# avaneev/r8brain-free-src

Measured on NVIDIA H100. Metric: input Msamples/s (Mrops), fp64 44100->96000, higher is better.
Workload: dtype f64

## Files before the change

### r8brain-free-src_b200/csrc/r8b_capi.cu

```cuda
#include "../../include/r8bgpu.h"

#include <algorithm>
#include <climits>
#include <cmath>
#include <cstddef>
#include <cstdio>
#include <cstdlib>
#include <cstring>
#include <functional>
#include <map>
#include <memory>
#include <optional>
#include <string>
#include <utility>
#include <vector>

#include "r8b_codec.cuh"
#include "r8b_dither.cuh"
#include "r8b_dsd.cuh"
#include "r8b_dsdmod.cuh"
#include "r8b_fft.cuh"
#include "r8b_hosttab.h"
#include "r8b_kernels.h"
#include "r8b_multi.h"
// ... 117 lines not shown
        return &h_;
    }

  private:
    H h_ = nullptr;
};
using Event = Handle<cudaEvent_t, cudaEventDestroy>;
using Stream = Handle<cudaStream_t, cudaStreamDestroy>;

template <class T>
struct RecRing {
    DevBuf<T> d;
    PinBuf<T> h[2];
    Event ev[2];
    int cur = 0;

    bool create(unsigned long long& charge, size_t n, const char* dev_what, const char* host_what, const char* ev_what)
    {
        if (!d.alloc(charge, n, dev_what)) return false;
        for (int k = 0; k < 2; k++)
            if (!h[k].alloc(n, host_what) || !cuda_ok(cudaEventCreateWithFlags(ev[k].put(), cudaEventDisableTiming), ev_what))
                return false;
        return true;
    }
    T* next(const char* what)
    {
        cur ^= 1;
        return cuda_ok(cudaEventSynchronize(ev[cur]), what) ? (T*) h[cur] : nullptr;
    }
    T* host() const { return h[cur]; }
    bool upload(size_t first, size_t n, cudaStream_t st, const char* what)
    {
        return cuda_ok(cudaMemcpyAsync(d + first, h[cur] + first, n * sizeof(T), cudaMemcpyHostToDevice, st), what) &&
               cuda_ok(cudaEventRecord(ev[cur], st), what);
    }
};

struct StageDev {
    int fft_log2 = 0, lg = 0, virt_up = 1;
    double nyq_gain = 0.0;
    DevBuf<double2> spec;
    DevBuf<double2> tw;
    bool large = false;
    DevBuf<double2> tw_m;
    DevBuf<double2> scratch;
    long long scratch_pairs = 0;
    DevBuf<double> bank;
    int frac_tile_fixed = 0;
    int frac_tile_ragged = 0;
    std::string unfused_variant;
    DevBuf<double> ring;
    long long ring_cap = 0;
    bool fused_with_next = false;
    bool fused_into_prev = false;
    DevBuf<int> phase_off;
    DevBuf<int> phase_row;
    DevBuf<double> gbank;
    DevBuf<int> goff;
    int gbank_len = 0, gbank_smem_len = 0, smaxp = 0, ir = 8;
    int yl = 0, yr = 0, ysh = 31, span_max = 0, bank_in_smem = 0;
    RecRing<int> ft_dp;
    RecRing<double> ft_fpos;
    int casc_len = 0;
    HbCascadeParams up_casc;
    int up_casc_smem = 0;
    int down_casc_len = 0;
    HbDownCascParams down_casc;
    int down_casc_smem = 0;
    int casc_variant = 0;
    DevBuf<double2> tw_tab;
    DevBuf<double2> c_tab;
    DevBuf<double2> cd_tab;
    DevBuf<double2> cs_tab;
    DevBuf<double2> c_tab_v1;
    bool bank_frag_order = false;
    bool f2_ok = false;
    bool f2_poly = false;
    bool f2_copy = false;
    FusedGeom fgeom;
    FusedVariant last_variant;
};

struct FusedKnobs {
    int f2_flags = 6;
    bool f2_flags_env = false;
    bool v1 = false;
    bool no_fusion = false;
    bool poly_v2 = false;
};

FusedKnobs fused_knobs_env()
{
    FusedKnobs k;
    if (const char* e = getenv("R8BGPU_F2_FLAGS")) {
        k.f2_flags = atoi(e);
        k.f2_flags_env = true;
    }
    k.v1 = getenv("R8BGPU_FUSED_V1") != nullptr;
    k.no_fusion = getenv("R8BGPU_NO_FUSION") != nullptr;
    k.poly_v2 = getenv("R8BGPU_POLY_V2") != nullptr;
    return k;
}

struct FusedPlan {
    FusedGeom geom;
    bool copy = false;
    bool poly_v2 = false;
    bool cs = false;
    bool whole = false;
    GroupBank tc, fma;
    bool tc_fits = false, fma_fits = false;
    bool tc_bank = false;
    bool bank_in_smem = false;
    int kernel = R8BGPU_FUSED_NONE;
};

FusedPlan plan_fused_stage(const std::vector<StageDesc>& st, size_t i, const FusedKnobs& k)
{
    FusedPlan fp;
    const StageDesc& s = st[i];
    if (s.kind != ST_BLOCKCONV) return fp;
    fp.whole = i + 1 < st.size() && st[i + 1].kind == ST_FRAC_WHOLE;
    if (fp.whole) {
        const StageDesc& f = st[i + 1];
        auto f2_fits = [](const GroupBank& gb) {
            return fused2_smem_bytes(gb.n_groups * gb.smaxp * gb.ir, false, false) <= kFused2SmemMax && gb.n_groups <= 192;
        };
        fp.tc = build_group_bank(f, 8, true);
        fp.fma = build_group_bank(f, choose_group_ir(f), false);
        fp.tc_fits = f2_fits(fp.tc);
        fp.fma_fits = f2_fits(fp.fma);
    }
    if (i + 1 < st.size() && !k.no_fusion) {
        fp.geom = fused_geometry(s, st[i + 1]);
        if (fp.geom.ok && fp.geom.up == 1 && (k.v1 || !(k.f2_flags & 4) || !fp.tc_fits)) fp.geom = FusedGeom();
    }
    const bool fused = fp.geom.ok;
    if (fused && st[i + 1].kind == ST_FRAC_POLY && fp.geom.up == 2 && (k.f2_flags & 4) && !k.v1 && k.poly_v2 &&
        (st[i + 1].bank.filter_len & 1) == 0 && st[i + 1].bank.filter_len <= 32)
        fp.poly_v2 = true;
    if (!fused && s.up == 2 && s.down == 1 && !s.block_exact && !k.no_fusion && !k.v1) {
        const BcTile bt = blockconv_tile(s);
        if (!bt.large && 2 * (4096 - 2 * bt.lg) >= 2048) fp.copy = true;
    }
    if ((fused && fp.geom.up == 2) || fp.copy) fp.cs = fused2_cs_fits(fused ? fused2_bank_doubles_max(st[i + 1]) : 0);
    if (fused && fp.whole) {
        const bool want_f2 = !k.v1;
        fp.tc_bank = want_f2 && (k.f2_flags & 4) && fp.tc_fits;
        const GroupBank& B = fp.tc_bank ? fp.tc : fp.fma;
        fp.bank_in_smem = fused_smem_bytes(B.n_groups * B.smaxp * B.ir) <= 220 * 1024;
        if (want_f2 && (fp.tc_bank || fp.fma_fits)) fp.kernel = fp.tc_bank ? R8BGPU_FUSED_F2_TC : R8BGPU_FUSED_F2_FMA;
        else fp.kernel = fp.bank_in_smem ? R8BGPU_FUSED_V1_SMEM : R8BGPU_FUSED_V1_GLOBAL;
    } else if (fused) {
        fp.kernel = R8BGPU_FUSED_ORDER2;
    } else if (fp.copy) {
        fp.kernel = R8BGPU_FUSED_F2_COPY;
    }
    return fp;
}

struct HbKnobs {
    bool no_cascade = false;
    bool no_last2 = false;
    int up_budget = 7000;
    int down_budget = 6400;
};

// ... 154 lines not shown
    std::vector<int> part_of, row_of;
    std::vector<std::vector<int>> chans;
    int max_out = 0, flush_max_out = 0;
    std::vector<Stream> streams;
    std::vector<Event> done;
    Event fork;
    RecRing<MapRec> map;
    DevBuf<unsigned char> raw_in;
    DevBuf<unsigned char> raw_out;
};

static_assert(sizeof(DitherCfg) == sizeof(r8bgpu_dither) && offsetof(DitherCfg, taps) == offsetof(r8bgpu_dither, taps),
              "DitherCfg mirrors r8bgpu_dither");
struct DitherState {
    std::vector<DitherCfg> cfg;
    bool any = false;
    DevBuf<DitherCfg> d_cfg;
    DevBuf<double> d_err;
    RecRing<DitherRec> rec;
    std::vector<long long> m;
    DevBuf<DitherCall> d_call;
    DevBuf<double> d_zero;
};

struct StateStaging {
    DevBuf<unsigned char> d_blob;
    PinBuf<unsigned char> h_blob;
    DevBuf<unsigned char> d_aux;
};

struct DsdOutState {
    DevBuf<DsdModState> d_state;
    std::vector<int> pend;
    RecRing<DsdModRec> rec;
    DevBuf<double> d_y;
    size_t y_cap = 0;
    DevBuf<unsigned char> d_in;
    DevBuf<unsigned char> d_bytes;
};

struct r8bgpu_batch {
    std::optional<DeviceGuard> releasing;
    unsigned long long dev_bytes = 0;
    std::unique_ptr<DsdOutState> dsd;
    std::unique_ptr<StateStaging> stx;
    std::unique_ptr<DitherState> dith;
    std::unique_ptr<ShardFront> front;
    std::unique_ptr<MixedFront> mixed;
    const Plan* plan = nullptr;
    Plan plan_copy;
    int n_ch = 0;
    int device = 0;
    cudaStream_t stream = nullptr;
    Schedule sched;
    bool diverged = false;
    RaggedSchedule rag;
    RecRing<RaggedRec> rec;
    bool links_fresh = false;
    std::vector<StageDev> dev;
    std::vector<StageCall> calls;
    unsigned long long launches = 0;
    bool timing = false;
    struct EvPair {
        int stage;
        Event a, b;
    };
    std::vector<EvPair> events;
    std::vector<double> stage_ms;
    std::vector<unsigned long long> stage_launches;
    DevBuf<double> st_in;
    DevBuf<double> st_out;
    DevBuf<unsigned char> raw_in;
    DevBuf<unsigned char> raw_out;
    DevBuf<double> fl_out;
    DevBuf<unsigned char> fl_raw;
    size_t fl_cap = 0;
    std::vector<long long> pass_n;
    std::vector<double> trim;
    Stream s_h2d, s_d2h, s_comp;
    int host_groups = 1;
    std::vector<Event> ev_h2d, ev_k;
    DevBuf<unsigned long long> prof;
    int n_sm = 0;
    int f2_flags = 6;
    bool f2_flags_env = false;
    unsigned long long prof_ctas = 0;
    bool prof_v2 = false;

    ~r8bgpu_batch()
    {
        if (front) {
            front->pool.reset();
            return;
        }
        releasing.emplace(device);
        if (mixed) {
            cudaStreamSynchronize(stream);
            mixed->parts.clear();
        }
        unsigned long long h[10] = {};
        if (prof != nullptr && cudaDeviceSynchronize() == cudaSuccess &&
            cudaMemcpy(h, prof, sizeof h, cudaMemcpyDeviceToHost) == cudaSuccess) {
            if (prof_v2) {
                const double n = prof_ctas ? (double) prof_ctas : 1.0;
                const unsigned long long tot = h[0] + h[1] + h[2] + h[3] + h[4] + h[7] + h[8];
                auto line = [&](const char* nm, double v) {
                    fprintf(stderr, "  %-26s %9.0f  (%4.1f %%)\n", nm, v / n, tot ? 100.0 * v / tot : 0.0);
                };
                fprintf(stderr, "[r8bgpu profile] k_up2_frac2 phases, mean clk per tile (one half-CTA) over %llu tiles:\n", prof_ctas);
                line("A_wait landed tile", (double) h[0]);
                line("A_work gather+fwd1", (double) h[1]);
                line("A_bar", (double) h[2]);
                line("B fwd2+fwd3", (double) h[3]);
                line("C+D split*G, inverse", (double) h[4]);
                line("E interp", (double) (h[7] + h[8]));
                line("  E_work mean over warps", h[5] / 8.0);
                line("  E_work max over warps", (double) h[6]);
                line("  E_bar (thread 0)", (double) h[7]);
                fprintf(stderr, "  %-26s %9.0f\n", "total", tot / n);
            } else {
                static const char* nm[8] = {"gather+fwd1", "fwd2", "fwd3", "C(split*G)", "inv1", "inv2", "inv3+ystore", "interp"};
                unsigned long long tot = 0;
                for (int i = 0; i < 8; i++) tot += h[i];
                fprintf(stderr, "[r8bgpu profile] k_up2_frac phases, mean clk per CTA over %llu CTAs:\n", prof_ctas);
                for (int i = 0; i < 8; i++)
                    fprintf(stderr, "  %-12s %9.0f  (%4.1f %%)\n", nm[i], prof_ctas ? (double) h[i] / prof_ctas : 0.0,
                            tot ? 100.0 * h[i] / tot : 0.0);
                if (h[8] + h[9] > 0)
                    fprintf(stderr, "  order-2 bank, clk per CTA: 4-output groups %.0f, queued single outputs %.0f\n",
                            (double) h[8] / prof_ctas, (double) h[9] / prof_ctas);
            }
        }
    }
};


static const std::vector<std::unique_ptr<r8bgpu_batch>>* sub_batches(const r8bgpu_batch* b)
{
    return b->front ? &b->front->shards : b->mixed ? &b->mixed->parts : nullptr;
}

static std::vector<const r8bgpu_batch*> plan_batches(const r8bgpu_batch* b)
{
    const auto* subs = sub_batches(b);
    if (subs == nullptr) return {b};
    std::vector<const r8bgpu_batch*> v;
    for (const auto& sb : *subs) v.push_back(sb.get());
    return v;
}

struct Slot {
    r8bgpu_batch* b;
    int row, sub;
};

static Slot slot_of(const r8bgpu_batch* b, int c)
{
    if (b->front) {
        const std::vector<int>& ch0 = b->front->ch0;
        const int s = (int) (std::upper_bound(ch0.begin(), ch0.end(), c) - ch0.begin()) - 1;
        return Slot{b->front->shards[(size_t) s].get(), c - ch0[(size_t) s], s};
    }
    if (b->mixed) {
        const int p = b->mixed->part_of[(size_t) c];
        return Slot{b->mixed->parts[(size_t) p].get(), b->mixed->row_of[(size_t) c], p};
    }
    return Slot{const_cast<r8bgpu_batch*>(b), c, 0};
}

struct ChannelGroup {
    r8bgpu_batch* b;
    std::vector<int> rows, idx;
};

static std::vector<ChannelGroup> group_channels(const r8bgpu_batch* b, const int* channels, int n)
{
    const auto* subs = sub_batches(b);
    std::vector<ChannelGroup> g(subs ? subs->size() : 1);
    for (size_t k = 0; k < g.size(); k++) g[k].b = subs ? (*subs)[k].get() : const_cast<r8bgpu_batch*>(b);
    for (int i = 0; i < n; i++) {
        const Slot s = slot_of(b, channels[i]);
        g[(size_t) s.sub].rows.push_back(s.row);
        g[(size_t) s.sub].idx.push_back(i);
    }
    return g;
}

template <class T>
static std::vector<T> gather(const T* v, const std::vector<int>& idx)
{
    std::vector<T> out;
    out.reserve(idx.size());
    for (int i : idx) out.push_back(v[i]);
    return out;
// ... 1314 lines not shown
                const double outs = 2.0 * p.span / ratio + 4.0;
                const int row_words = 6 * p.flen;
                p.poly_row_stride = 3 * p.flen + ((row_words % 8) == 4 ? 0 : 2);
                const int cap = (224 * 1024 - fused_smem_bytes(0) - fused_poly_queue_bytes()) /
                                (p.poly_row_stride * (int) sizeof(double));
                const double up = fr * p.fracs * outs + 4.0, dn = (1.0 - fr) * p.fracs * outs + 4.0;
                const double need = up < dn ? up : dn;
                const int chunks = (int) ceil(need / cap);
                if (cap >= 8 && chunks <= 4) {
                    p.poly_dir = up < dn ? 1 : -1;
                    p.poly_rows_cap = cap;
                    p.poly_chunks = chunks < 1 ? 1 : chunks;
                    const long long nn = llround(ratio);
                    if (nn >= 1 && nn <= 3 && !getenv("R8BGPU_POLY_SINGLE")) {
                        p.poly_n = (int) nn;
                        p.ysh = 4;
                    }
                }
            }
            if (p.poly_chunks < 1) p.poly_chunks = 1;
            if (b->prof == nullptr && getenv("R8BGPU_PROFILE") && b->prof.alloc(b->dev_bytes, 10, "profile: cudaMalloc"))
                cudaMemset(b->prof, 0, 10 * sizeof(unsigned long long));
            p.prof = b->prof;
#ifdef R8BGPU_EXPERIMENTS
            if (const char* e = getenv("R8BGPU_DEBUG")) p.debug = atoi(e);
#endif
            if (b->prof) {
                b->prof_ctas += (unsigned long long) (v2 ? p.n_tiles : (p.n_tiles + 1) / 2) * nch;
                b->prof_v2 = v2;
            }
            if (v2) {
                p.n_ch = nch;
                p.flags = b->f2_flags;
                p.tw_tab = d.tw_tab;
                p.c_tab = d.c_tab;
                p.cd_tab = d.cd_tab;
                p.cs_tab = d.cs_tab;
                p.up = d.fgeom.up;
                p.ylen = d.fgeom.up * 4096;
                if (!fd.bank_frag_order) p.flags &= ~4;
                if (!b->f2_flags_env && !v2_poly && p.up != 1 && p.cs_tab != nullptr && (p.flags & 4)) p.flags |= 1;
                const bool cs = p.cs_tab != nullptr;
                p.stage_off = (p.ir == 8 && !(p.flags & 4) && fused2_smem_bytes(p.gbank_smem_len, cs, true) <= kFused2SmemMax &&
                               !getenv("R8BGPU_NO_STAGE")) ? fused2_stage_off(p.gbank_smem_len, cs) : 0;
                if (v2_poly) {
                    p.ysh = 31;
                    p.gbank_smem_len = 0;
                    p.stage_off = 0;
                }
                p.glog = v2_poly ? 0 : fused2_choose_glog(p.span, f.in_step, f.out_step, p.ir);
                p.mbu = v2_poly ? 0 : fused2_choose_mbu(p.span, f.in_step, f.out_step);
                launch_up2_frac2(p, src, dst, b->n_sm, st, &b->dev[i].last_variant);
            } else {
                p.c_tab = d.c_tab_v1;
                launch_up2_frac(p, src, dst, nch, st, &b->dev[i].last_variant);
            }
            b->launches++;
        } else
        switch (s.kind) {
        case ST_BLOCKCONV: {
            if (d.f2_copy) {
                FusedParams fp;
                memset(&fp, 0, sizeof fp);
                fp.mode = 2;
                fp.e0 = c.e0;
                fp.e1 = c.e1;
                fp.p_lo = c.e0 & ~1LL;
                fp.p_hi = c.e1;
                fused2_tiles(fp, d.fgeom, i == 0 ? (int) (c.n0 & 1) : -1);
                fp.lg = d.lg;
                fp.ysh = 31;
                fp.spec = d.spec;
                fp.tw = d.tw;
                fp.tw_tab = d.tw_tab;
                fp.c_tab = d.c_tab;
                fp.cd_tab = d.cd_tab;
                fp.cs_tab = d.cs_tab;
                fp.up = 2;
                fp.ylen = 8192;
                fp.ir = 8;
                fp.out_step = 8;
                fp.smaxp = 4;
                fp.n_ch = nch;
                fp.flags = b->f2_flags & 2;
                launch_up2_frac2(fp, src, dst, b->n_sm, st, &b->dev[i].last_variant);
                b->launches++;
                break;
            }
            BlockConvParams p;
            blockconv_call_fields(p, s, d.virt_up, d.lg, d.fft_log2, c.e0, c.e1);
            p.nyq_gain = d.nyq_gain;
            p.spec = d.spec;
            p.tw = d.tw;
            if (d.large) {
                BcLargeParams lp;
                lp.bc = p;
                lp.tw_m = d.tw_m;
                lp.scratch = d.scratch;
                const long long pairs = (p.n_tiles + 1) / 2;
                lp.group_ch = (int) std::max(1LL, std::min((long long) nch, d.scratch_pairs / std::max(1LL, pairs)));
                b->launches += (unsigned long long) launch_blockconv_large(lp, src, dst, nch, st);
                if (p.n_tiles > 0 && nch > 0)
                    b->dev[i].unfused_variant = bcl_variant(p, lp.group_ch, nch);
                break;
            }
            launch_blockconv(p, src, dst, nch, st);
            if (p.n_tiles > 0 && nch > 0) b->dev[i].unfused_variant = blockconv_variant(p);
            b->launches++;
            break;
        }
        case ST_FRAC_WHOLE:
        case ST_FRAC_POLY: {
            FracParams p;
            memset(&p, 0, sizeof p);
            p.flen = s.bank.filter_len;
            p.fll = s.bank.filter_len / 2 - 1;
            p.e0 = c.e0;
            p.e1 = c.e1;
            p.bank = d.bank;
            p.in_step = s.in_step;
            p.out_step = s.out_step;
            p.fracs = s.bank.fracs;
            p.ssr = s.kind == ST_FRAC_POLY ? c.ssr : s.src_rate;
            p.dsr = s.kind == ST_FRAC_POLY ? c.dsr : s.dst_rate;
            p.in_counter0 = c.in_counter0;
            p.in_pos_int0 = c.in_pos_int0;
            p.in_pos_shift = c.in_pos_shift;
            p.fpos0 = c.fpos0;
            p.p0 = c.p0;
            p.pos_dp = d.ft_dp.d;
            p.pos_fpos = d.ft_fpos.d;
            const int tile = d.frac_tile_fixed > 0 ? d.frac_tile_fixed : frac_tile(p.ssr / p.dsr, p.flen);
            if (s.kind == ST_FRAC_WHOLE) launch_frac_whole(p, tile, src, dst, nch, st);
            else launch_frac_poly(p, tile, src, dst, nch, st);
            if (p.e1 > p.e0 && nch > 0) b->dev[i].unfused_variant = frac_variant(s, tile);
            b->launches++;
            break;
        }
        case ST_HBUP:
        case ST_HBDOWN: {
            HbParams p;
            memset(&p, 0, sizeof p);
            p.ntaps = s.hb_taps;
            p.e0 = c.e0;
            p.e1 = c.e1;
            for (int k = 0; k < s.hb_taps; k++) p.taps[k] = s.hb[(size_t) k];
            if (s.kind == ST_HBUP) launch_hbup(p, src, dst, nch, st);
            else launch_hbdown(p, src, dst, nch, st);
            b->launches++;
            break;
        }
        }
        time_end(b, ev, st);
    }
    if (l > 0) {
        const StageCall& c0 = calls[0];
        const StageDev& d0 = b->dev[0];
        long long from = c0.n1 - d0.ring_cap;
        if (from < c0.n0) from = c0.n0;
        launch_save_tail(d_in, (long long) in_stride, c0.n0, from, c0.n1, d0.ring + (long long) ch0 * d0.ring_cap, d0.ring_cap,
                         d0.ring_cap - 1, nch, st, tio.in_fmt, tio.in_scale);
        b->launches++;
    }
}


static bool has_fasttiming(const Plan& P)
// ... 2983 lines not shown
```

### r8brain-free-src_b200/csrc/r8b_fused2.cu

```cuda
#include "r8b_kernels.h"

#include <algorithm>
#include <cstdint>
#include <type_traits>

#include "r8b_fused2_core.cuh"
#include "r8b_poly.cuh"

namespace r8bgpu {

namespace {

using namespace f2;

constexpr int NT2 = 2 * HT;
constexpr int STAGE_UP = fft_pad(FN);

__device__ __forceinline__ void bar_half(int h) { asm volatile("bar.sync %0, 256;" ::"r"(h + 1) : "memory"); }
__device__ __forceinline__ uint32_t smem_u32(const void* p) { return (uint32_t) __cvta_generic_to_shared(p); }
__device__ __forceinline__ void mbar_init(unsigned long long* b, int count)
{
    asm volatile("mbarrier.init.shared::cta.b64 [%0], %1;" ::"r"(smem_u32(b)), "r"(count) : "memory");
}
__device__ __forceinline__ void fence_mbar_init() { asm volatile("fence.mbarrier_init.release.cluster;" ::: "memory"); }
// ... 39 lines not shown
    const int n_j = s_i[0], c_cnt = s_i[1], jshift = s_i[2];
    const int n_groups = (p.out_step + 7) / 8;
    const int n_gt = (n_groups + G::GL - 1) / G::GL;
    const int gt = task % n_gt, chunk = task / n_gt;
    const int wrow = (lane ^ ((lane >> 2) & 1)) * 8, wsw = (lane >> 1) & 3;
#pragma unroll
    for (int q = 0; q < IQ2; q++) {
        const int cq = chunk * G::CYC + q * G::CL;
        if (cq > c_cnt) break;
#pragma unroll
        for (int i = 0; i < 4; i++)
            *reinterpret_cast<double2*>(stg + wrow + 2 * (i ^ wsw)) = make_double2(acc[2 * i][q], acc[2 * i + 1][q]);
        __syncwarp();
        const int ci = lane & 3;
#pragma unroll
        for (int t = 0; t < 4; t++) {
            const int R = (lane & ~3) + t;
            const double2 v = *reinterpret_cast<const double2*>(stg + (R ^ ((R >> 2) & 1)) * 8 + 2 * (ci ^ ((R >> 1) & 3)));
            const int c = cq + (R & (G::CL - 1));
            const int grp = gt * G::GL + (R >> (5 - GLOG));
            if (c > c_cnt || grp >= n_groups) continue;
            const int r0 = p.delta + grp * 8;
            const int j = c * p.out_step + r0 + jshift + 2 * ci;
            double* o = s_o + j;
            const bool in0 = (p.wrap || r0 + 2 * ci < p.out_step) && j >= 0 && j < n_j;
            const bool in1 = (p.wrap || r0 + 2 * ci + 1 < p.out_step) && j + 1 >= 0 && j + 1 < n_j;
            if (in0 && in1 && ((reinterpret_cast<unsigned long long>(o) & 15) == 0)) {
                *reinterpret_cast<double2*>(o) = v;
            } else {
                if (in0) o[0] = v.x;
                if (in1) o[1] = v.y;
            }
        }
        __syncwarp();
    }
}

}

__device__ __forceinline__ void dmma884(double& c0, double& c1, double a, double b)
{
    asm volatile("mma.sync.aligned.m8n8k4.row.col.f64.f64.f64.f64 {%0,%1}, {%2}, {%3}, {%0,%1};" : "+d"(c0), "+d"(c1) : "d"(a), "d"(b));
}

template <int KW>
__device__ __forceinline__ void dmma16(double (&c)[4], const double (&a)[KW / 2], const double (&b)[KW / 4])
{
    if constexpr (KW == 16)
        asm volatile("mma.sync.aligned.m16n8k16.row.col.f64.f64.f64.f64 {%0,%1,%2,%3}, {%4,%5,%6,%7,%8,%9,%10,%11}, "
                     "{%12,%13,%14,%15}, {%0,%1,%2,%3};"
                     : "+d"(c[0]), "+d"(c[1]), "+d"(c[2]), "+d"(c[3])
                     : "d"(a[0]), "d"(a[1]), "d"(a[2]), "d"(a[3]), "d"(a[4]), "d"(a[5]), "d"(a[6]), "d"(a[7]), "d"(b[0]), "d"(b[1]),
                       "d"(b[2]), "d"(b[3]));
    else if constexpr (KW == 8)
        asm volatile("mma.sync.aligned.m16n8k8.row.col.f64.f64.f64.f64 {%0,%1,%2,%3}, {%4,%5,%6,%7}, {%8,%9}, {%0,%1,%2,%3};"
                     : "+d"(c[0]), "+d"(c[1]), "+d"(c[2]), "+d"(c[3])
                     : "d"(a[0]), "d"(a[1]), "d"(a[2]), "d"(a[3]), "d"(b[0]), "d"(b[1]));
    else
        asm volatile("mma.sync.aligned.m16n8k4.row.col.f64.f64.f64.f64 {%0,%1,%2,%3}, {%4,%5}, {%6}, {%0,%1,%2,%3};"
                     : "+d"(c[0]), "+d"(c[1]), "+d"(c[2]), "+d"(c[3])
                     : "d"(a[0]), "d"(a[1]), "d"(b[0]));
}

template <int IRV, bool PADV, int GLOG, bool TC, int UP = 2, bool COPY = false, bool POLY = false, bool CS = false, bool LIN = false>
__global__ void __launch_bounds__(NT2, 1) k_up2_frac2(const __grid_constant__ FusedParams p, const __grid_constant__ SrcView src,
                                                      const __grid_constant__ DstView dst)
{
    extern __shared__ __align__(128) double2 smem[];
    double2* const tw2 = smem + 2 * FPL2;
    double2* const twf = tw2 + 256;
    double* const sbank = reinterpret_cast<double*>(twf + 256);
    const int n_groups = (p.out_step + IRV - 1) / IRV, esz = p.smaxp * IRV;
    const int n_bank = (COPY || POLY) ? 0 : n_groups;
    static_assert(!CS || UP == 2, "the symmetric spectrum table is the 2x pair's");
    double2* const scs = reinterpret_cast<double2*>(sbank + ((n_bank * esz + 1) & ~1));
    TileEntry* const tab = reinterpret_cast<TileEntry*>(reinterpret_cast<char*>(smem) + p.tab_off);
    __shared__ __align__(8) unsigned long long mb[5];
    __shared__ TileEntry s_te[2];
    __shared__ int s_goff[192];

    const int tid = threadIdx.x, h = tid >> 8, ht = tid & (HT - 1), lane = tid & 31, wh = ht >> 5;
    double2* const buf = smem + h * FPL2;
    const int n_units = p.n_tiles * p.n_ch;
    const bool pingpong = (p.flags & 1) != 0, tma_in = (p.flags & 2) != 0;

    if (tid == 0) {
#pragma unroll
        for (int i = 0; i < 5; i++) mbar_init(&mb[i], 1);
        fence_mbar_init();
    }
    if (!COPY && !POLY && tid < n_groups) s_goff[tid] = __ldg(&p.goff[p.delta + tid * IRV]);
    if (!COPY)
        for (int i = tid; i < p.n_tab; i += NT2) tab[i] = tile_entry(p, dst.base, i);
    __syncthreads();
    if (tid == 0) {
        mbar_expect_tx(&mb[0], (uint32_t) (512 * sizeof(double2) + (size_t) n_bank * esz * sizeof(double) +
                                           (CS ? CS_PAIRS * sizeof(double2) : 0)));
        bulk_g2s(tw2, p.tw_tab, 512 * sizeof(double2), &mb[0]);
        if (CS) bulk_g2s(scs, p.cs_tab, CS_PAIRS * sizeof(double2), &mb[0]);
        for (int g = 0; g < n_bank; g++)
            bulk_g2s(sbank + g * esz, p.gbank + (long long) (p.delta + g * IRV) * esz, (uint32_t) (esz * sizeof(double)), &mb[0]);
        mbar_arrive(&mb[3]);
    }

    const int stride = 2 * (int) gridDim.x;
    int u = 2 * (int) blockIdx.x + h;
    uint32_t par_in = 0, par_turn = 0;
    Tile t;
    int path = -1;
    auto tile_src = [&](const Tile& tt) { return tile_run(src, tt); };
    if (u < n_units) {
        t = tile_of(p, u);
        path = tile_input_path(src, t);
        if (path == 2 && !tma_in) path = 1;
        if (path == 2 && ht == 0) {
            mbar_expect_tx(&mb[1 + h], FM * sizeof(double));
            bulk_g2s(buf + STAGE_UP, tile_src(t), FM * sizeof(double), &mb[1 + h]);
        }
    }
    mbar_wait(&mb[0], 0);

#ifdef R8BGPU_PHASE_TIMERS
    __shared__ unsigned long long s_emax[2];
    if (ht == 0) s_emax[h] = 0;
    long long t_prev = clock64();
#define R8B_TICK(i)                                                                  \
    if (p.prof != nullptr && ht == 0) {                                              \
        const long long t_now = clock64();                                           \
        atomicAdd(&p.prof[i], (unsigned long long) (t_now - t_prev));                \
        t_prev = t_now;                                                              \
    }
#else
#define R8B_TICK(i)
#endif
    for (; u < n_units; u += stride) {
        Tile tn = t;
        int pathn = -1;
        if (u + stride < n_units) {
            tn = tile_of(p, u + stride);
            pathn = tile_input_path(src, tn);
            if (pathn == 2 && !tma_in) pathn = 1;
            if ((pathn == 1 || pathn == 2) && ht == 0) bulk_prefetch_l2(reinterpret_cast<const void*>(reinterpret_cast<unsigned long long>(tile_src(tn)) & ~15ull),
                                                        FM * sizeof(double));
        }
        {
            double2 v[8];
            if (path == 2) {
                R8B_TICK(1)
                mbar_wait(&mb[1 + h], par_in);
                R8B_TICK(0)
                par_in ^= 1;
                const double2* st = buf + STAGE_UP;
#pragma unroll
                for (int j = 0; j < 8; j++) v[j] = st[ht + 256 * j];
            } else {
                gather_tile(v, src, t, path, ht);
            }
            fwd_pass1_r8(v, buf, tw2, twf, ht);
        }
        if (!COPY && u - t.ch * p.n_tiles >= p.n_tab && ht == HT - 1) s_te[h] = tile_entry(p, dst.base, u - t.ch * p.n_tiles);
        R8B_TICK(1)
        bar_half(h);
        R8B_TICK(2)
        constexpr bool fuse_c = (UP == 2);
        if (ht < FN / 16) {
            fwd_pass<256>(buf, tw2, ht);
            __syncwarp();
            if constexpr (fuse_c) fwd_pass16_skew(buf, ht);
            else fwd_pass<16>(buf, tw2, ht);
        }
        bar_half(h);
        R8B_TICK(3)
        if constexpr (fuse_c) {
            double2 z1[8], z2[8];
            cd1_load(buf, ht, z1, z2);
            bar_half(h);
            if constexpr (CS) cd1s_compute(scs, __ldg(&p.cs_tab[CS_PAIRS + ht]), __ldg(&p.cs_tab[CS_PAIRS + HT + ht]), buf, ht, z1, z2);
            else cd1_compute(p, buf, ht, z1, z2);
        } else {
            double2 z1[4], z2[4], ze = make_double2(0.0, 0.0);
            c_load(buf, ht, z1, z2);
            if (ht == 0) ze = buf[fft_pad(slot_of<FN>(FN / 2))];
            bar_half(h);
#pragma unroll
            for (int i = 0; i < 4; i++) c1_pair_tab(p, buf, ht, i, z1[i], z2[i]);
            if (ht == 0) c1_pair_mid(p, buf, ze);
            bar_half(h);
        }
        if constexpr (UP == 2) {
            __syncwarp();
            inv_pass<256>(buf, tw2, ht);
            bar_half(h);
            {
                double2 v[16];
                inv3_load(buf, tw2, twf, ht, v);
                bar_half(h);
                y_store<PADV>(buf, v, ht, t.w, p.ysh);
            }
        } else {
            if (ht < FN / 16) {
                inv_pass<16>(buf, tw2, ht);
                __syncwarp();
                inv_pass<256>(buf, tw2, ht);
            }
            bar_half(h);
            {
                double2 v[8];
                inv1_last_load(buf, tw2, twf, ht, v);
                bar_half(h);
                y_store1<PADV>(buf, v, ht, t.w, p.ysh);
            }
        }
        bar_half(h);
        R8B_TICK(4)
        if (pingpong) {
            mbar_wait(&mb[3 + h], par_turn);
            par_turn ^= 1;
        }
#ifdef R8BGPU_PHASE_TIMERS
        const long long t_e0 = clock64();
#endif
        {
            const double* yb = reinterpret_cast<const double*>(buf);
            const int ti = u - t.ch * p.n_tiles;
            const TileEntry& te = ti < p.n_tab ? tab[ti] : s_te[h];
            const int* si = te.s;
            const long long drow = (long long) t.ch * dst.stride;
            if constexpr (POLY) {
                const int ka = si[0], kb = si[1], N = p.poly_n, flen = p.flen, ksteps = (flen + 3) >> 2;
                const int row = lane >> 2, kq = lane & 3;
                const unsigned full = 0xffffffffu;
                const int n_rounds = (kb - ka + 31) >> 5;
                int cached_row = -2;
                double bq[8];
                auto load_b = [&](int fmin) {
                    cached_row = fmin;
                    int brow = fmin + (row & 1);
                    if (brow > p.fracs) brow = p.fracs;
                    const double* __restrict__ br = p.bank + (long long) brow * 3 * flen + (row >> 1);
#pragma unroll
                    for (int ks = 0; ks < 8; ks++) {
// ... 98 lines not shown
                    for (int i = ht; i < cnt; i += HT) orow[(d0 + i) & dst.mask] = yb[off + i];
                }
            } else if constexpr (TC) {
                MmaTile mt;
                mt.load(te, drow);
                const int n_mu = mt.n_j > 0 ? mma_units(p, mt.c_cnt) : 0, smaxp = p.smaxp;
                double* const so = dst.ptr + drow + (te.off & dst.mask);
                constexpr int WS = HT / 32;
                auto run_units = [&](auto mb_tag) {
                    constexpr int MB = decltype(mb_tag)::value;
                    MmaUnit mu;
                    mu.set(wh, n_groups);
                    for (int unit = wh; unit < n_mu; unit += WS) {
                        int yo[2 * MB];
                        const int goff = s_goff[mu.g];
#pragma unroll
                        for (int i = 0; i < 2 * MB; i++) yo[i] = mma_a_index(p, mt, mu, goff, i, lane);
                        const double* const gb = sbank + mma_b_index(p, mu, lane);
                        double acc[MB][4];
#pragma unroll
                        for (int m = 0; m < MB; m++) acc[m][0] = acc[m][1] = acc[m][2] = acc[m][3] = 0.0;
                        auto kchunk = [&](auto kw_tag, int k0) {
                            constexpr int KW = decltype(kw_tag)::value;
                            double b[KW / 4];
#pragma unroll
                            for (int i = 0; i < KW / 4; i++) b[i] = gb[8 * k0 + 32 * i];
#pragma unroll
                            for (int m = 0; m < MB; m++) {
                                double a[KW / 2];
#pragma unroll
                                for (int i = 0; i < KW / 2; i++) {
                                    const int yi = yo[2 * m + (i & 1)] + k0 + 4 * (i >> 1);
                                    a[i] = PADV ? yb[ylay(yi, p.ysh)] : yb[yi];
                                }
                                dmma16<KW>(acc[m], a, b);
                            }
                        };
                        using K16 = std::integral_constant<int, 16>;
                        const int k16 = smaxp & ~15;
#pragma unroll 1
                        for (int k0 = 0; k0 < k16; k0 += 16) kchunk(K16(), k0);
                        if (smaxp & 8) kchunk(std::integral_constant<int, 8>(), k16);
                        if (smaxp & 4) kchunk(std::integral_constant<int, 4>(), k16 + (smaxp & 8));
#pragma unroll
                        for (int m = 0; m < MB; m++) {
                            mma_store<LIN>(p, dst, t.ch, mt, so, mu, 2 * m, lane, acc[m][0], acc[m][1]);
                            mma_store<LIN>(p, dst, t.ch, mt, so, mu, 2 * m + 1, lane, acc[m][2], acc[m][3]);
                        }
                        mu.advance(WS, n_groups);
                    }
                };
                switch (mma_mbu(p)) {
                case 2: run_units(std::integral_constant<int, 1>()); break;
                case 4: run_units(std::integral_constant<int, 2>()); break;
                default: run_units(std::integral_constant<int, 3>()); break;
                }
            } else if (si[0] > 0) {
                const int n_tasks = TaskGeom<IRV, GLOG>::n_tasks(p, si[1]);
                double* const stg = p.stage_off > 0 ? reinterpret_cast<double*>(smem) + p.stage_off + (tid >> 5) * 256 : nullptr;
                double* const so = dst.ptr + drow + (te.off & dst.mask);
                for (int task = wh; task < n_tasks; task += HT / 32) {
                    TaskGeom<IRV, GLOG> g;
                    g.set(p, s_goff, task, lane);
                    int yo[IQ2];
                    interp_windows<IRV, GLOG>(p, g, si, yo);
                    double acc[IRV][IQ2];
                    interp_acc<IRV, PADV>(yb, sbank + g.grp * esz, yo, p.smaxp, p.ysh, acc);
                    if (IRV == 8 && dst.mask == -1 && stg != nullptr) {
                        if constexpr (IRV == 8) interp_store_staged<GLOG>(p, si, so, stg, task, lane, acc);
                    } else {
                        interp_store_direct<IRV, GLOG>(p, dst, t.ch, g, si, so, acc);
                    }
                }
            }
        }
#ifdef R8BGPU_PHASE_TIMERS
        if (p.prof != nullptr && lane == 0) {
            const unsigned long long dt = (unsigned long long) (clock64() - t_e0);
            atomicAdd(&p.prof[5], dt);
            atomicMax(&s_emax[h], dt);
        }
#endif
        R8B_TICK(8)
        bar_half(h);
        R8B_TICK(7)
#ifdef R8BGPU_PHASE_TIMERS
        if (p.prof != nullptr && ht == 0) {
            atomicAdd(&p.prof[6], s_emax[h]);
            s_emax[h] = 0;
        }
#endif
        if (ht == 0) {
            if (pingpong) mbar_arrive(&mb[4 - h]);
            if (pathn == 2) {
                fence_proxy_async();
                mbar_expect_tx(&mb[1 + h], FM * sizeof(double));
                bulk_g2s(buf + STAGE_UP, tile_src(tn), FM * sizeof(double), &mb[1 + h]);
            }
        }
        t = tn;
        path = pathn;
    }
#undef R8B_TICK
}

template <int IRV, bool PADV, int GLOG, bool TC = false, int UP = 2, bool COPY = false, bool POLY = false, bool CS = false,
          bool LIN = false>
static void launch_inst2(const FusedParams& p, const SrcView& src, const DstView& dst, int grid, int smem, cudaStream_t st,
                         FusedVariant* v)
{
    ensure_dyn_smem<k_up2_frac2<IRV, PADV, GLOG, TC, UP, COPY, POLY, CS, LIN>>(227 * 1024);
    k_up2_frac2<IRV, PADV, GLOG, TC, UP, COPY, POLY, CS, LIN><<<(unsigned) grid, NT2, smem, st>>>(p, src, dst);
    if (v != nullptr) {
        *v = FusedVariant();
        v->kernel = 2;
        v->ir = IRV;
        v->pad = PADV;
        v->glog = GLOG;
        v->tc = TC;
        v->up = UP;
        v->copy = COPY;
        v->poly = POLY;
        v->cs = CS;
        v->lin = LIN;
        v->mbu = p.mbu;
    }
}

template <bool PADV, int UP, bool CS>
static void launch_tc(const FusedParams& p, const SrcView& src, const DstView& dst, int grid, int smem, cudaStream_t st,
                      FusedVariant* v)
{
    if (dst.fmt == FMT_F64 && dst.mask == -1) launch_inst2<8, PADV, 0, true, UP, false, false, CS, true>(p, src, dst, grid, smem, st, v);
    else launch_inst2<8, PADV, 0, true, UP, false, false, CS>(p, src, dst, grid, smem, st, v);
}

template <bool CS>
static void launch_f2(const FusedParams& p, const SrcView& src, const DstView& dst, int grid, int smem, cudaStream_t st,
                      FusedVariant* v)
{
    const bool pad = p.ysh != 31;
#define R8B_F2_CASE(IRV, GL)                                                              \
    if (pad) launch_inst2<IRV, true, GL, false, 2, false, false, CS>(p, src, dst, grid, smem, st, v); \
    else launch_inst2<IRV, false, GL, false, 2, false, false, CS>(p, src, dst, grid, smem, st, v);
    if (p.mode == 1) {
        launch_inst2<8, false, 0, true, 2, false, true, CS>(p, src, dst, grid, smem, st, v);
        return;
    }
    if (p.mode == 2) {
        launch_inst2<8, false, 0, true, 2, true, false, CS>(p, src, dst, grid, smem, st, v);
        return;
    }
    if (p.up == 1) {
        if constexpr (!CS) {
            if (pad) launch_tc<true, 1, false>(p, src, dst, grid, smem, st, v);
            else launch_tc<false, 1, false>(p, src, dst, grid, smem, st, v);
        }
    } else if (p.ir == 8 && (p.flags & 4)) {
        if (pad) launch_tc<true, 2, CS>(p, src, dst, grid, smem, st, v);
        else launch_tc<false, 2, CS>(p, src, dst, grid, smem, st, v);
    } else if (p.ir == 10) {
        if (p.glog == 2) { R8B_F2_CASE(10, 2) } else if (p.glog == 1) { R8B_F2_CASE(10, 1) } else { R8B_F2_CASE(10, 0) }
    } else {
        if (p.glog == 2) { R8B_F2_CASE(8, 2) } else if (p.glog == 1) { R8B_F2_CASE(8, 1) } else { R8B_F2_CASE(8, 0) }
    }
#undef R8B_F2_CASE
}

void launch_up2_frac2(const FusedParams& p, const SrcView& src, const DstView& dst, int n_sm, cudaStream_t st, FusedVariant* v)
{
    const int n_units = p.n_tiles * p.n_ch;
    if (n_units <= 0) return;
    int grid = (n_units + 1) / 2;
    if (grid > n_sm) grid = n_sm;
    const bool cs = p.up != 1 && p.cs_tab != nullptr;
    FusedParams q = p;
    int smem = fused2_smem_bytes(p.gbank_smem_len, cs, p.stage_off > 0);
    q.tab_off = smem;
    q.n_tab = p.mode == 2 ? 0 : std::max(0, std::min(p.n_tiles, (kFused2SmemMax - smem) / (int) sizeof(TileEntry)));
    smem += q.n_tab * (int) sizeof(TileEntry);
// ... 6 lines not shown
```

### r8brain-free-src_b200/csrc/r8b_fused2_core.cuh

```cuda
#pragma once
#include <climits>

#include "r8b_fused_common.cuh"
#include "r8b_poly.cuh"

namespace r8bgpu {
namespace f2 {

constexpr int FN = 2048;
constexpr int FPL2 = FPL + 16;
constexpr int SKEW0 = fft_padded_len(FN);
constexpr int HT = 256;
constexpr int IQ2 = 3;

struct Tile {
    int ch;
    long long A0, A1;
    long long w;
};

R8B_HD Tile tile_of(const FusedParams& p, int u)
{
    Tile t;
    t.ch = u / p.n_tiles;
    const int ti = u - t.ch * p.n_tiles;
    t.A0 = p.p_lo + (long long) ti * p.span;
    t.A1 = t.A0 + p.span;
    if (t.A1 > p.p_hi) t.A1 = p.p_hi;
    t.w = (p.up == 1 ? t.A0 - p.yl : (t.A0 - p.yl) / 2) - p.lg;
    return t;
}

R8B_HD const double* tile_run(const SrcView& src, const Tile& t)
{
    if (t.w >= src.cur_base && t.w + FM <= src.avail)
        return src.cur_fmt == FMT_F64 ? src.cur + (long long) t.ch * src.cur_stride + (t.w - src.cur_base) : nullptr;
    if (t.w >= 0 && t.w + FM <= src.avail && t.w + FM <= src.cur_base) {
        const long long i0 = t.w & src.ring_mask;
        if (i0 + FM <= src.ring_mask + 1) return src.ring + (long long) t.ch * src.ring_stride + i0;
    }
    return nullptr;
}

R8B_HD int tile_input_path(const SrcView& src, const Tile& t)
{
    if (src.cur_fmt != FMT_F64 && t.w >= src.cur_base && t.w + FM <= src.avail) return 3;
    const double* a = tile_run(src, t);
    if (a == nullptr) return 0;
    return (reinterpret_cast<unsigned long long>(a) & 15) == 0 ? 2 : 1;
}

R8B_HD void gather_tile(double2 (&v)[8], const SrcView& src, const Tile& t, int path, int r)
{
    if (path == 3) {
        const long long i0 = (long long) t.ch * src.cur_stride + (t.w - src.cur_base) + 2 * r;
#pragma unroll
        for (int j = 0; j < 8; j++)
            v[j] = make_double2(typed_load(src.cur, i0 + 512 * j, src.cur_fmt, src.cur_scale),
                                typed_load(src.cur, i0 + 512 * j + 1, src.cur_fmt, src.cur_scale));
    } else if (path != 0) {
        const double* __restrict__ a = tile_run(src, t) + 2 * r;
        if ((reinterpret_cast<unsigned long long>(a) & 15) == 0) {
#pragma unroll
            for (int j = 0; j < 8; j++) v[j] = R8B_LDG(reinterpret_cast<const double2*>(a + 512 * j));
        } else {
#pragma unroll
            for (int j = 0; j < 8; j++) v[j] = make_double2(R8B_LDG(a + 512 * j), R8B_LDG(a + 512 * j + 1));
        }
    } else {
#pragma unroll
        for (int j = 0; j < 8; j++) {
            const long long n = t.w + 2 * (r + 256 * j);
            v[j] = make_double2(src_read_f(src, t.ch, n), src_read_f(src, t.ch, n + 1));
        }
    }
}

R8B_HD void fwd_pass1_r8(double2 (&v)[8], double2* __restrict__ s, const double2* __restrict__ twc,
                         const double2* __restrict__ twf, int r)
{
    Network<8, +1>::run(v);
    const double2 w1 = tw_pair(twc, twf, r, 2), w2 = tw_pair(twc, twf, r, 4), w4 = tw_pair(twc, twf, r, 8);
    const double2 w3 = cprod(w1, w2);
    s[fft_pad(r)] = v[0];
    s[fft_pad(r + 1 * 256)] = cmul<+1>(v[bitrev<8>(1)], w1);
    s[fft_pad(r + 2 * 256)] = cmul<+1>(v[bitrev<8>(2)], w2);
    s[fft_pad(r + 3 * 256)] = cmul<+1>(v[bitrev<8>(3)], w3);
    s[fft_pad(r + 4 * 256)] = cmul<+1>(v[bitrev<8>(4)], w4);
    s[fft_pad(r + 5 * 256)] = cmul<+1>(v[bitrev<8>(5)], cprod(w1, w4));
    s[fft_pad(r + 6 * 256)] = cmul<+1>(v[bitrev<8>(6)], cprod(w2, w4));
    s[fft_pad(r + 7 * 256)] = cmul<+1>(v[bitrev<8>(7)], cprod(w3, w4));
}

R8B_HD int c_freq(int ht, int u) { return freq_of<FN>(16 * ((ht >> 3) + 32 * u) + (ht & 7)); }

R8B_HD void c_load(const double2* __restrict__ buf, int ht, double2 (&z1)[4], double2 (&z2)[4])
{
#pragma unroll
    for (int u = 0; u < 4; u++) {
        const int s1 = 16 * ((ht >> 3) + 32 * u) + (ht & 7);
        const int k = freq_of<FN>(s1);
        const int s2 = slot_of<FN>((FN - k) & (FN - 1));
        z1[u] = buf[fft_pad(s1)];
        z2[u] = buf[fft_pad(s2)];
    }
}

R8B_HD int skew(int slot) { return slot + (slot >> 4) + (slot >> 7); }

R8B_HD void fwd_pass16_skew(double2* __restrict__ buf, int g)
{
    double2 v[16];
#pragma unroll
    for (int j = 0; j < 16; j++) v[j] = buf[fft_pad(16 * g + j)];
    Network<16, +1>::run(v);
#pragma unroll
    for (int q = 0; q < 16; q++) buf[SKEW0 + skew(16 * g + q)] = v[bitrev<16>(q)];
}

R8B_HD void cd1_load(const double2* __restrict__ buf, int g, double2 (&z1)[8], double2 (&z2)[8])
{
    const int k0 = (g >> 4) + 16 * (g & 15);
#pragma unroll
    for (int t = 0; t < 8; t++) {
        const int k = k0 + 256 * t;
        z1[t] = buf[SKEW0 + skew(slot_of<FN>(k))];
        z2[t] = buf[SKEW0 + skew(slot_of<FN>((FN - k) & (FN - 1)))];
    }
}

template <int T>
R8B_HD void cd1_bin(const FusedParams& p, int g, double2 w0, double2 z1, double2 z2, double2 (&v)[16])
{
    const double2 a = make_double2(z1.x + z2.x, z1.y - z2.y);
    const double2 b = make_double2(z1.y + z2.y, z2.x - z1.x);
    const double2 wb = cmul<+1>(b, mul_root<16, T, +1>(w0));
    const double2 x0 = make_double2(a.x + wb.x, a.y + wb.y);
    const double2 x1 = make_double2(a.x - wb.x, a.y - wb.y);
    v[T] = cmul<+1>(x0, R8B_LDG(&p.cd_tab[T * HT + g]));
    v[T + 8] = cmul<+1>(x1, R8B_LDG(&p.cd_tab[(T + 8) * HT + g]));
}

R8B_HD void cd1_compute(const FusedParams& p, double2* __restrict__ buf, int g, const double2 (&z1)[8], const double2 (&z2)[8])
{
    const double2 w0 = R8B_LDG(&p.cd_tab[16 * HT + g]);
    double2 v[16];
    cd1_bin<0>(p, g, w0, z1[0], z2[0], v);
    cd1_bin<1>(p, g, w0, z1[1], z2[1], v);
    cd1_bin<2>(p, g, w0, z1[2], z2[2], v);
    cd1_bin<3>(p, g, w0, z1[3], z2[3], v);
    cd1_bin<4>(p, g, w0, z1[4], z2[4], v);
    cd1_bin<5>(p, g, w0, z1[5], z2[5], v);
    cd1_bin<6>(p, g, w0, z1[6], z2[6], v);
    cd1_bin<7>(p, g, w0, z1[7], z2[7], v);
    Network<16, -1>::run(v);
#pragma unroll
    for (int j = 0; j < 16; j++) buf[fft_pad(16 * g + j)] = v[bitrev<16>(j)];
}

constexpr int CS_PAIRS = FN + 1;
R8B_HD int cs_entry(int k) { return (k & ~255) | ((k & 15) << 4) | ((k >> 4) & 15); }
R8B_HD int cs_second(int g) { return cs_entry(FN - ((g >> 4) + 16 * (g & 15))); }

template <int T>
R8B_HD double2 rot32(double2 a)
{
    if constexpr ((T & 1) == 0) {
        return mul_root<16, T / 2, -1>(a);
    } else {
        constexpr double c1 = 0.98078528040323044913, s1 = 0.19509032201612826785;
        constexpr double c3 = 0.83146961230254523708, s3 = 0.55557023301960222474;
        constexpr double c = T == 1 ? c1 : T == 3 ? c3 : T == 5 ? s3 : s1;
        constexpr double s = T == 1 ? s1 : T == 3 ? s3 : T == 5 ? c3 : c1;
        return make_double2(fma(a.x, c, -a.y * s), fma(a.x, s, a.y * c));
// ... 382 lines not shown
```

Measured before the change: 57420.

## Software-pipeline next tile gather and fwd pass1 into registers before half-barrier

Restructures the fused up2-frac2 kernel so the next tile's input is gathered and run through the first radix-8 FFT pass in registers at the end of the current iteration, then only stored to shared memory at the start of the next. Non-landing variants default to the register path, with the ping-pong mbarrier arrive moved per warp. The TMA bulk-copy path is no longer opt-in via the flag, since the default flags drop bit 2 and bit 2 is no longer read. Aligned input loads also switch to L1 no-allocate non-coherent loads. The aim is to hide global load latency behind the interpolation stage, at the cost of extra live registers across the loop.

```diff
diff --git a/r8brain-free-src_b200/csrc/r8b_capi.cu b/r8brain-free-src_b200/csrc/r8b_capi.cu
--- a/r8brain-free-src_b200/csrc/r8b_capi.cu
+++ b/r8brain-free-src_b200/csrc/r8b_capi.cu
@@ -223,7 +223,7 @@
 };
 
 struct FusedKnobs {
-    int f2_flags = 6;
+    int f2_flags = 4;
     bool f2_flags_env = false;
     bool v1 = false;
     bool no_fusion = false;
@@ -544,7 +544,7 @@
     std::vector<Event> ev_h2d, ev_k;
     DevBuf<unsigned long long> prof;
     int n_sm = 0;
-    int f2_flags = 6;
+    int f2_flags = 4;
     bool f2_flags_env = false;
     unsigned long long prof_ctas = 0;
     bool prof_v2 = false;
@@ -570,8 +570,8 @@
                     fprintf(stderr, "  %-26s %9.0f  (%4.1f %%)\n", nm, v / n, tot ? 100.0 * v / tot : 0.0);
                 };
                 fprintf(stderr, "[r8bgpu profile] k_up2_frac2 phases, mean clk per tile (one half-CTA) over %llu tiles:\n", prof_ctas);
-                line("A_wait landed tile", (double) h[0]);
-                line("A_work gather+fwd1", (double) h[1]);
+                line("A_next gather / landing", (double) h[0]);
+                line("A_work fwd1 stores", (double) h[1]);
                 line("A_bar", (double) h[2]);
                 line("B fwd2+fwd3", (double) h[3]);
                 line("C+D split*G, inverse", (double) h[4]);
@@ -2052,7 +2052,6 @@
                 fp.out_step = 8;
                 fp.smaxp = 4;
                 fp.n_ch = nch;
-                fp.flags = b->f2_flags & 2;
                 launch_up2_frac2(fp, src, dst, b->n_sm, st, &b->dev[i].last_variant);
                 b->launches++;
                 break;
diff --git a/r8brain-free-src_b200/csrc/r8b_fused2.cu b/r8brain-free-src_b200/csrc/r8b_fused2.cu
--- a/r8brain-free-src_b200/csrc/r8b_fused2.cu
+++ b/r8brain-free-src_b200/csrc/r8b_fused2.cu
@@ -145,11 +145,13 @@
     const int tid = threadIdx.x, h = tid >> 8, ht = tid & (HT - 1), lane = tid & 31, wh = ht >> 5;
     double2* const buf = smem + h * FPL2;
     const int n_units = p.n_tiles * p.n_ch;
-    const bool pingpong = (p.flags & 1) != 0, tma_in = (p.flags & 2) != 0;
+    const bool pingpong = (p.flags & 1) != 0;
+    constexpr bool LAND = UP == 2 && !CS;
+    constexpr int TURN = LAND ? 1 : HT / 32;
 
     if (tid == 0) {
 #pragma unroll
-        for (int i = 0; i < 5; i++) mbar_init(&mb[i], 1);
+        for (int i = 0; i < 5; i++) mbar_init(&mb[i], i >= 3 ? TURN : 1);
         fence_mbar_init();
     }
     if (!COPY && !POLY && tid < n_groups) s_goff[tid] = __ldg(&p.goff[p.delta + tid * IRV]);
@@ -163,25 +165,33 @@
         if (CS) bulk_g2s(scs, p.cs_tab, CS_PAIRS * sizeof(double2), &mb[0]);
         for (int g = 0; g < n_bank; g++)
             bulk_g2s(sbank + g * esz, p.gbank + (long long) (p.delta + g * IRV) * esz, (uint32_t) (esz * sizeof(double)), &mb[0]);
-        mbar_arrive(&mb[3]);
+        for (int i = 0; i < TURN; i++) mbar_arrive(&mb[3]);
     }
 
     const int stride = 2 * (int) gridDim.x;
     int u = 2 * (int) blockIdx.x + h;
     uint32_t par_in = 0, par_turn = 0;
+    auto input_path = [&](const Tile& tt) {
+        const int pa = tile_input_path(src, tt);
+        return LAND && pa == 1 && (reinterpret_cast<unsigned long long>(tile_run(src, tt)) & 15) == 0 ? 2 : pa;
+    };
     Tile t;
     int path = -1;
-    auto tile_src = [&](const Tile& tt) { return tile_run(src, tt); };
+    double2 vn[8];
     if (u < n_units) {
         t = tile_of(p, u);
-        path = tile_input_path(src, t);
-        if (path == 2 && !tma_in) path = 1;
-        if (path == 2 && ht == 0) {
-            mbar_expect_tx(&mb[1 + h], FM * sizeof(double));
-            bulk_g2s(buf + STAGE_UP, tile_src(t), FM * sizeof(double), &mb[1 + h]);
+        path = input_path(t);
+        if (path == 2) {
+            if (ht == 0) {
+                mbar_expect_tx(&mb[1 + h], FM * sizeof(double));
+                bulk_g2s(buf + STAGE_UP, tile_run(src, t), FM * sizeof(double), &mb[1 + h]);
+            }
+        } else {
+            gather_tile(vn, src, t, path, ht);
         }
     }
     mbar_wait(&mb[0], 0);
+    if (u < n_units && path != 2) fwd_pass1_r8_regs(vn, tw2, twf, ht);
 
 #ifdef R8BGPU_PHASE_TIMERS
     __shared__ unsigned long long s_emax[2];
@@ -201,25 +211,22 @@
         int pathn = -1;
         if (u + stride < n_units) {
             tn = tile_of(p, u + stride);
-            pathn = tile_input_path(src, tn);
-            if (pathn == 2 && !tma_in) pathn = 1;
-            if ((pathn == 1 || pathn == 2) && ht == 0) bulk_prefetch_l2(reinterpret_cast<const void*>(reinterpret_cast<unsigned long long>(tile_src(tn)) & ~15ull),
-                                                        FM * sizeof(double));
-        }
-        {
-            double2 v[8];
-            if (path == 2) {
-                R8B_TICK(1)
-                mbar_wait(&mb[1 + h], par_in);
-                R8B_TICK(0)
-                par_in ^= 1;
-                const double2* st = buf + STAGE_UP;
-#pragma unroll
-                for (int j = 0; j < 8; j++) v[j] = st[ht + 256 * j];
-            } else {
-                gather_tile(v, src, t, path, ht);
-            }
-            fwd_pass1_r8(v, buf, tw2, twf, ht);
+            pathn = input_path(tn);
+            if ((pathn == 1 || pathn == 2) && ht == 0)
+                bulk_prefetch_l2(reinterpret_cast<const void*>(reinterpret_cast<unsigned long long>(tile_run(src, tn)) & ~15ull),
+                                 FM * sizeof(double));
+        }
+        if (path == 2) {
+            R8B_TICK(1)
+            mbar_wait(&mb[1 + h], par_in);
+            R8B_TICK(0)
+            par_in ^= 1;
+            const double2* st = buf + STAGE_UP;
+#pragma unroll
+            for (int j = 0; j < 8; j++) vn[j] = st[ht + 256 * j];
+            fwd_pass1_r8(vn, buf, tw2, twf, ht);
+        } else {
+            fwd_pass1_r8_store(vn, buf, ht);
         }
         if (!COPY && u - t.ch * p.n_tiles >= p.n_tab && ht == HT - 1) s_te[h] = tile_entry(p, dst.base, u - t.ch * p.n_tiles);
         R8B_TICK(1)
@@ -484,6 +491,18 @@
         }
 #endif
         R8B_TICK(8)
+        if (!LAND && pingpong) {
+            __syncwarp();
+            if (lane == 0) mbar_arrive(&mb[4 - h]);
+        }
+        if (pathn >= 0 && pathn != 2) {
+            gather_tile(vn, src, tn, pathn, ht);
+            fwd_pass1_r8_regs(vn, tw2, twf, ht);
+        } else {
+#pragma unroll
+            for (int j = 0; j < 8; j++) vn[j] = make_double2(0.0, 0.0);
+        }
+        R8B_TICK(0)
         bar_half(h);
         R8B_TICK(7)
 #ifdef R8BGPU_PHASE_TIMERS
@@ -493,11 +512,11 @@
         }
 #endif
         if (ht == 0) {
-            if (pingpong) mbar_arrive(&mb[4 - h]);
+            if (LAND && pingpong) mbar_arrive(&mb[4 - h]);
             if (pathn == 2) {
                 fence_proxy_async();
                 mbar_expect_tx(&mb[1 + h], FM * sizeof(double));
-                bulk_g2s(buf + STAGE_UP, tile_src(tn), FM * sizeof(double), &mb[1 + h]);
+                bulk_g2s(buf + STAGE_UP, tile_run(src, tn), FM * sizeof(double), &mb[1 + h]);
             }
         }
         t = tn;
diff --git a/r8brain-free-src_b200/csrc/r8b_fused2_core.cuh b/r8brain-free-src_b200/csrc/r8b_fused2_core.cuh
--- a/r8brain-free-src_b200/csrc/r8b_fused2_core.cuh
+++ b/r8brain-free-src_b200/csrc/r8b_fused2_core.cuh
@@ -45,9 +45,18 @@
 R8B_HD int tile_input_path(const SrcView& src, const Tile& t)
 {
     if (src.cur_fmt != FMT_F64 && t.w >= src.cur_base && t.w + FM <= src.avail) return 3;
-    const double* a = tile_run(src, t);
-    if (a == nullptr) return 0;
-    return (reinterpret_cast<unsigned long long>(a) & 15) == 0 ? 2 : 1;
+    return tile_run(src, t) == nullptr ? 0 : 1;
+}
+
+R8B_HD double2 ld_input2(const double2* a)
+{
+#ifdef __CUDA_ARCH__
+    double2 v;
+    asm("ld.global.nc.L1::no_allocate.v2.f64 {%0, %1}, [%2];" : "=d"(v.x), "=d"(v.y) : "l"(a));
+    return v;
+#else
+    return *a;
+#endif
 }
 
 R8B_HD void gather_tile(double2 (&v)[8], const SrcView& src, const Tile& t, int path, int r)
@@ -62,7 +71,7 @@
         const double* __restrict__ a = tile_run(src, t) + 2 * r;
         if ((reinterpret_cast<unsigned long long>(a) & 15) == 0) {
 #pragma unroll
-            for (int j = 0; j < 8; j++) v[j] = R8B_LDG(reinterpret_cast<const double2*>(a + 512 * j));
+            for (int j = 0; j < 8; j++) v[j] = ld_input2(reinterpret_cast<const double2*>(a + 512 * j));
         } else {
 #pragma unroll
             for (int j = 0; j < 8; j++) v[j] = make_double2(R8B_LDG(a + 512 * j), R8B_LDG(a + 512 * j + 1));
@@ -76,20 +85,35 @@
     }
 }
 
-R8B_HD void fwd_pass1_r8(double2 (&v)[8], double2* __restrict__ s, const double2* __restrict__ twc,
-                         const double2* __restrict__ twf, int r)
+R8B_HD void fwd_pass1_r8_regs(double2 (&v)[8], const double2* __restrict__ twc, const double2* __restrict__ twf, int r)
 {
     Network<8, +1>::run(v);
     const double2 w1 = tw_pair(twc, twf, r, 2), w2 = tw_pair(twc, twf, r, 4), w4 = tw_pair(twc, twf, r, 8);
     const double2 w3 = cprod(w1, w2);
-    s[fft_pad(r)] = v[0];
-    s[fft_pad(r + 1 * 256)] = cmul<+1>(v[bitrev<8>(1)], w1);
-    s[fft_pad(r + 2 * 256)] = cmul<+1>(v[bitrev<8>(2)], w2);
-    s[fft_pad(r + 3 * 256)] = cmul<+1>(v[bitrev<8>(3)], w3);
-    s[fft_pad(r + 4 * 256)] = cmul<+1>(v[bitrev<8>(4)], w4);
-    s[fft_pad(r + 5 * 256)] = cmul<+1>(v[bitrev<8>(5)], cprod(w1, w4));
-    s[fft_pad(r + 6 * 256)] = cmul<+1>(v[bitrev<8>(6)], cprod(w2, w4));
-    s[fft_pad(r + 7 * 256)] = cmul<+1>(v[bitrev<8>(7)], cprod(w3, w4));
+    double2 o[8];
+    o[0] = v[0];
+    o[1] = cmul<+1>(v[bitrev<8>(1)], w1);
+    o[2] = cmul<+1>(v[bitrev<8>(2)], w2);
+    o[3] = cmul<+1>(v[bitrev<8>(3)], w3);
+    o[4] = cmul<+1>(v[bitrev<8>(4)], w4);
+    o[5] = cmul<+1>(v[bitrev<8>(5)], cprod(w1, w4));
+    o[6] = cmul<+1>(v[bitrev<8>(6)], cprod(w2, w4));
+    o[7] = cmul<+1>(v[bitrev<8>(7)], cprod(w3, w4));
+#pragma unroll
+    for (int j = 0; j < 8; j++) v[j] = o[j];
+}
+
+R8B_HD void fwd_pass1_r8_store(const double2 (&v)[8], double2* __restrict__ s, int r)
+{
+#pragma unroll
+    for (int j = 0; j < 8; j++) s[fft_pad(r + j * 256)] = v[j];
+}
+
+R8B_HD void fwd_pass1_r8(double2 (&v)[8], double2* __restrict__ s, const double2* __restrict__ twc,
+                         const double2* __restrict__ twf, int r)
+{
+    fwd_pass1_r8_regs(v, twc, twf, r);
+    fwd_pass1_r8_store(v, s, r);
 }
 
 R8B_HD int c_freq(int ht, int u) { return freq_of<FN>(16 * ((ht >> 3) + 32 * u) + (ht & 7)); }
```

New measurement: 58830 (median of 6 runs). +2.5%, better.
